# illini-robomaster/irmv_detection

Hardware: AMD Instinct MI355X
Metric: end-to-end FPS (preprocess→NMS→PnP) 640×640 YOLOv8n, 1/2/4/8 MI355X (higher is better)
Workload: dtype f16

## Files before the change

irmv_detection_amd/_build.py:

```python
from __future__ import annotations

import os
import shutil
import subprocess

_HERE = os.path.dirname(os.path.abspath(__file__))
CSRC = os.path.join(_HERE, "csrc")
LIB_DIR = os.path.join(_HERE, "lib")
LIB_PATH = os.path.join(LIB_DIR, "libirmv_hip.so")
INCLUDE = os.path.join(os.path.dirname(_HERE), "include")

SOURCES = [
    ("k_pre.hip", []),
    ("k_front.hip", []),
    ("k_c2f.hip", []),
    ("k_bneck.hip", []),
    ("k_kpt.hip", []),
    ("k_conv.hip", []),
    ("k_post.hip", ["-ffp-contract=off"]),
    ("k_light.hip", ["-ffp-contract=off"]),
    ("k_shuffle.hip", []),
    ("engine.cpp", ["-x", "hip"]),
]
COMMON = ["-O3", "-std=c++17", "-fPIC", "--offload-arch=gfx950", "-Wall", "-Wno-unused-function",
          "-mllvm", "-amdgpu-mfma-vgpr-form", "-I", INCLUDE]


def source_hash() -> str:
    import hashlib
    h = hashlib.sha256()
    names = sorted(set([s for s, _ in SOURCES] + ["irmv_common.hpp", "pnp_device.hpp", "numa.hpp"]))
    for n in names:
        pth = os.path.join(CSRC, n)
        if os.path.exists(pth):
            h.update(n.encode() + b"\0" + open(pth, "rb").read())
    h.update(open(os.path.join(INCLUDE, "irmv_hip.h"), "rb").read())
    h.update(" ".join(COMMON[:-2]).encode())
    for src, extra in SOURCES:
        h.update((src + " " + " ".join(extra)).encode())
    return h.hexdigest()


def hipcc() -> str:
    for cand in (shutil.which("hipcc"), "/opt/rocm/bin/hipcc"):
        if cand and os.path.exists(cand):
            return cand
    raise RuntimeError("hipcc not found: the HIP extension cannot be built")


def _stale(target: str, deps) -> bool:
    if not os.path.exists(target):
        return True
    t = os.path.getmtime(target)
    return any(os.path.getmtime(d) > t for d in deps)


COMM_PATH = os.path.join(LIB_DIR, "libirmv_comm.so")


def build_comm(force: bool = False, verbose: bool = False) -> str:
    os.makedirs(LIB_DIR, exist_ok=True)
    src = os.path.join(CSRC, "comm.cpp")
    deps = [src, os.path.join(INCLUDE, "irmv_comm.h"), os.path.join(INCLUDE, "irmv_hip.h"), __file__]
    if force or _stale(COMM_PATH, deps):
        rocm_lib = os.path.join(os.path.dirname(os.path.dirname(os.path.realpath(hipcc()))), "lib")
        cmd = [hipcc(), "-O2", "-std=c++17", "-fPIC", "-shared", "-Wall", "-I", INCLUDE, src, "-o", COMM_PATH,
               "-L", rocm_lib, "-lrccl", "-Wl,-rpath," + rocm_lib]
        if verbose:
            print(" ".join(cmd))
        subprocess.check_call(cmd)
    return COMM_PATH


def build(force: bool = False, verbose: bool = False) -> str:
    os.makedirs(LIB_DIR, exist_ok=True)
    headers = [os.path.join(CSRC, "irmv_common.hpp"), os.path.join(CSRC, "pnp_device.hpp"), os.path.join(CSRC, "numa.hpp"), os.path.join(INCLUDE, "irmv_hip.h"), __file__]
    objs = []
    cc = hipcc()
    for src, extra in SOURCES:
        sp = os.path.join(CSRC, src)
        obj = os.path.join(LIB_DIR, os.path.splitext(src)[0] + ".o")
        if force or _stale(obj, [sp] + headers):
            cmd = [cc] + COMMON + extra + os.environ.get("IRMV_EXTRA_HIPCC_FLAGS", "").split() + ["-c", sp, "-o", obj]
            if verbose:
                print(" ".join(cmd))
            subprocess.check_call(cmd)
        objs.append(obj)
    if force or _stale(LIB_PATH, objs):
        cmd = [cc, "-shared", "-fPIC", "--offload-arch=gfx950", "-o", LIB_PATH] + objs
        if verbose:
            print(" ".join(cmd))
        subprocess.check_call(cmd)
    return LIB_PATH


if __name__ == "__main__":
    print(build(force=False, verbose=True))
    print(build_comm(force=False, verbose=True))
# ... 1 lines not shown
```

irmv_detection_amd/csrc/engine.cpp:

```cpp
#include <hip/hip_runtime.h>

#include <algorithm>
#include <chrono>
#include <cmath>
#include <cstdio>
#include <cstring>
#include <fstream>
#include <map>
#include <mutex>
#include <set>
#include <memory>
#include <string>
#include <vector>

#include "../../include/irmv_hip.h"
#include "irmv_common.hpp"
#include "numa.hpp"

using namespace irmv;

constexpr int kLightPointsCap = 4096;

static thread_local std::string g_err;
static int fail(int code, const std::string &msg)
// ... 19 lines not shown
        snprintf(buf, sizeof buf, "irmv_hip 0.3 (gfx950; HIP runtime %d)", v);
    });
    return buf;
}
extern "C" int irmv_device_synchronize(int device)
{
    HIP_TRY(hipSetDevice(device));
    HIP_TRY(hipDeviceSynchronize());
    return IRMV_OK;
}
extern "C" int irmv_device_count(int *count)
{
    if (!count) return fail(IRMV_ERR_ARG, "count is null");
    HIP_TRY(hipGetDeviceCount(count));
    return IRMV_OK;
}

#pragma pack(push, 1)
struct BlobHeader { char magic[4]; uint32_t version, nc, nk, reg_max, n_layers, dtype, reserved; };
struct BlobLayer { char name[32]; uint32_t cin, cout, k, stride, act, pad; uint64_t w_off, b_off; };
#pragma pack(pop)

struct LayerW {
    std::string name;
    int cin, cout, k, stride, act;
    int groups;
    const uint16_t *w;
    const float *b;
};

static float half_bits_to_float(uint16_t h)
{
    const uint32_t sign = ((uint32_t)h & 0x8000u) << 16;
    uint32_t exp = (h >> 10) & 0x1fu, man = h & 0x3ffu, x;
    if (exp == 0) {
        if (man == 0) x = sign;
        else {
            int e = -1;
            do { e++; man <<= 1; } while (!(man & 0x400u));
            x = sign | ((uint32_t)(112 - e) << 23) | ((man & 0x3ffu) << 13);
        }
    } else if (exp == 31) x = sign | 0x7f800000u | (man << 13);
    else x = sign | ((exp + 112u) << 23) | (man << 13);
    float f;
    memcpy(&f, &x, 4);
    return f;
}

static uint16_t float_to_half_bits(float f)
{
    uint32_t x;
    memcpy(&x, &f, 4);
    const uint32_t sign = (x >> 16) & 0x8000u;
    x &= 0x7fffffffu;
    if (x >= 0x7f800000u) return (uint16_t)(sign | 0x7c00u | ((x > 0x7f800000u) ? 0x200u : 0u));
    if (x >= 0x477ff000u) return (uint16_t)(sign | 0x7c00u);
    if (x < 0x33000001u) return (uint16_t)sign;
    if (x < 0x38800000u) {
        const int shift = 126 - (int)(x >> 23);
        const uint32_t man = (x & 0x7fffffu) | 0x800000u;
        uint32_t h = man >> shift;
        const uint32_t rem = man & ((1u << shift) - 1u), half = 1u << (shift - 1);
        if (rem > half || (rem == half && (h & 1u))) h++;
        return (uint16_t)(sign | h);
    }
    uint32_t h = ((x >> 23) - 112u) << 10 | ((x >> 13) & 0x3ffu);
    const uint32_t rem = x & 0x1fffu;
    if (rem > 0x1000u || (rem == 0x1000u && (h & 1u))) h++;
    return (uint16_t)(sign | h);
}

struct Tensor {
    std::string name;
    void *base = nullptr;
    size_t slot_elems = 0;
    int H = 0, W = 0, C = 0;
    bool f32 = false;
    size_t esize() const { return f32 ? 4 : 2; }
    void *slot(int s) const { return static_cast<char *>(base) + (size_t)s * slot_elems * esize(); }
};

struct SegRef { int t = -1, coff = 0, C = 0, shift = 0; };

enum OpKind { OP_PRE, OP_CONV0, OP_CONV, OP_POOL, OP_NMS, OP_LIGHT, OP_FRONT, OP_C2F2, OP_C2F32, OP_DW, OP_SHUF, OP_SCAN, OP_BNECK, OP_KPT3 };

struct Op {
    OpKind kind;
    std::string layer;
    ConvCfg cfg{};
    ConvCfg cfg_one{};
    char kname_one[48] = {0};
    SegRef s0, s1;
    int Hin = 0, Win = 0, Hout = 0, Wout = 0, cin = 0, cout = 0, cout_pad = 0, ksteps = 0;
    int out_t = -1, out_coff = 0, res_t = -1, res_coff = 0;
    half_t *w_packed = nullptr;
    half_t *w_k16 = nullptr;
    half_t *w_lds[4] = {nullptr, nullptr, nullptr, nullptr};
    float *bias = nullptr;
    double flops = 0, bytes = 0;
    double w_bytes = 0;
    double out_bytes = 0;
    bool pair = false;
    int lane = 0;
    int level = -1;
    int signal = -1;
    char kname[48] = {0};
    int sub[4] = {-1, -1, -1, -1};
    int mode = 0;
    bool shortcut = false;
    int fuse_next = -1;
    bool fused_away = false;
    int group = -1;
    int bneck = -1;
    int kpt3 = -1;
};

struct GraphKey {
    int first, count;
    uint32_t flags;
    bool operator<(const GraphKey &o) const
    {
        return std::tie(first, count, flags) < std::tie(o.first, o.count, o.flags);
    }
};

struct SlotGroup {
    int first = 0, count = 0;
    hipEvent_t h2d = nullptr, out = nullptr;
    hipStream_t compute = nullptr;
    bool in_flight = false;
    bool async_up = false;
};

struct irmv_engine {
    irmv_engine_cfg cfg{};
    int nc = 0, nk = 0, A = 0, no = 0;
    int backbone = 0;
    int num_cus = 256;
    int numa_node = -1;
    bool numa_placed = false;
    struct HeadGroup { std::vector<int> members; int family = 0, nt = 1; ConvCfg cfg{}; char name[48] = {0}; };
    std::vector<HeadGroup> head_groups;
    bool post_keys_only = false;
    bool emit_scan = false;
    int emit_level_abase[3] = {0, 0, 0};
    bool split_scan = true;
    int *cand_counts = nullptr;
    int lvl_hw[3] = {0, 0, 0}, lvl_base[3] = {0, 0, 0};
    size_t frame_bytes = 0;
    hipStream_t stream = nullptr;
    hipStream_t extra_streams[7] = {nullptr, nullptr, nullptr, nullptr, nullptr, nullptr, nullptr};
    int num_streams = 1;
    hipStream_t h2d_stream = nullptr;
    std::map<std::pair<int, int>, SlotGroup> groups;
    std::vector<SlotGroup *> slot_owner;
    bool inline_copies = false;
    bool graph_upload = true;
    uint8_t *src_host = nullptr;
    int sync_launch = 0;
    hipStream_t enq_stream = nullptr;
    uint8_t *src_host_dev = nullptr;
    int upload_kernel_blocks = 256;
    uint8_t *src_dev = nullptr;
    uint8_t *rot_dev = nullptr;
    AxisTap *tap_x = nullptr, *tap_y = nullptr;
    std::vector<Tensor> tensors;
    std::map<std::string, int> tensor_idx;
    std::vector<Op> ops;
    std::vector<void *> dev_allocs;
    int head_t[3] = {-1, -1, -1};
    float *head_all = nullptr;
    PnpConst *pnp_dev = nullptr;
    long long *dbg_dev = nullptr;
    std::set<std::string> lazy_tensors;
    bool fused_front = false;
    int front_tiles_x = 0, front_tiles_y = 0, front_stage_bytes = 0, front_tile_y = kFrontTileY;
    int front_v[4] = {0, 0, 0, 0};
    int front_fastx = 0, front_fx_i0 = 0, front_fx_step = 2;
    bool classical = false;
    signed char *light_labels = nullptr;
    size_t light_pool = 0;
    short *light_points = nullptr, *light_hulls = nullptr;
    float *light_boxes = nullptr;
    DevDet *light_dets_dev = nullptr, *light_dets_host = nullptr;
    float *boxes = nullptr;
    unsigned long long *keys = nullptr;
    DevDet *dets_dev = nullptr, *dets_host = nullptr, *dets_host_dev = nullptr;
    DevFrameOut *fout_dev = nullptr, *fout_host = nullptr, *fout_host_dev = nullptr;
    bool zero_copy_results = false;
    half_t *conv0_w = nullptr;
    float *conv0_b = nullptr;
    PostArgs post{};
    std::map<GraphKey, hipGraphExec_t> graphs;
    double last_detect_ms = 0;
    std::vector<uint8_t> blob;
    std::vector<LayerW> layers;
    std::vector<std::vector<uint16_t>> dequant;
// ... 575 lines not shown
    TRY(new_tensor(e, "6", s16, s16, 128, false, &a6));
    TRY(new_tensor(e, "7", s32, s32, 256, false, &a7));
    TRY(new_tensor(e, "8", s32, s32, 256, false, &a8));
    TRY(new_tensor(e, "9.cat", s32, s32, 512, false, &s9));
    TRY(new_tensor(e, "9", s32, s32, 256, false, &a9));
    TRY(new_tensor(e, "12", s16, s16, 128, false, &a12));
    TRY(new_tensor(e, "15", s8, s8, 64, false, &a15));
    TRY(new_tensor(e, "16", s16, s16, 64, false, &a16));
    TRY(new_tensor(e, "18", s16, s16, 128, false, &a18));
    TRY(new_tensor(e, "19", s32, s32, 128, false, &a19));
    TRY(new_tensor(e, "21", s32, s32, 256, false, &a21));

    { Op op; op.kind = OP_PRE; op.layer = "preprocess"; snprintf(op.kname, sizeof op.kname, "preprocess");
      op.bytes = (double)e->frame_bytes + (double)net * net * 8; e->ops.push_back(op); }
    {
        const LayerW *l = find_layer(e, "model.0.conv");
        if (!l || l->cin != 3 || l->cout != 16 || l->k != 3 || l->stride != 2)
            return fail(IRMV_ERR_MODEL, "model.0.conv missing or not 3x3 s2 3->16");
        std::vector<uint16_t> w(2 * 64 * 8, 0);
        std::vector<float> b(16);
        for (int o = 0; o < 16; o++) b[o] = (float)((double)l->b[o] * (double)kActScale);
        for (int ks = 0; ks < 2; ks++)
            for (int lane = 0; lane < 64; lane++)
                for (int j = 0; j < 8; j++) {
                    const int g = lane >> 4, o = lane & 15;
                    const int kh = 2 * ks + (g >> 1), kw = 2 * (g & 1) + (j >> 2), ci = j & 3;
                    if (kh < 3 && kw < 3 && ci < 3) w[((size_t)ks * 64 + lane) * 8 + j] = l->w[(o * 9 + kh * 3 + kw) * 3 + ci];
                }
        TRY(dev_alloc(e, (void **)&e->conv0_w, w.size() * 2));
        TRY(dev_alloc(e, (void **)&e->conv0_b, b.size() * 4));
        HIP_TRY(hipMemcpy(e->conv0_w, w.data(), w.size() * 2, hipMemcpyHostToDevice));
        HIP_TRY(hipMemcpy(e->conv0_b, b.data(), b.size() * 4, hipMemcpyHostToDevice));
        Op op; op.kind = OP_CONV0; op.layer = "model.0.conv"; snprintf(op.kname, sizeof op.kname, "conv0_mfma");
        op.flops = 2.0 * s2 * s2 * 16 * 27;
        op.bytes = (double)net * net * 8 + (double)s2 * s2 * 32 + 27 * 16 * 2;
        e->ops.push_back(op);
    }
    TRY(add_conv(e, "model.1.conv", SegRef{a0, 0, 16, 0}, SegRef{}, s2, s2, a1, 0));
    {
        const Op &m1 = e->ops.back();
        if (!(m1.cfg.cin16 && m1.ksteps == 5 && m1.pair && m1.cout_pad == 32 && m1.out_coff == 0)) e->fused_front = false;
        if (e->fused_front) {
            Op op; op.kind = OP_FRONT; op.layer = "preprocess+model.0+model.1"; snprintf(op.kname, sizeof op.kname, "front_fused");
            op.flops = e->ops[1].flops + m1.flops;
            op.bytes = (double)e->frame_bytes + (double)s4 * s4 * 32 * 2;
            op.w_packed = m1.w_packed; op.bias = m1.bias; op.out_t = m1.out_t;
            for (Op &o : e->ops) o.fused_away = true;
            e->lazy_tensors.insert("input"); e->lazy_tensors.insert("0");
            e->ops.push_back(op);
        }
    }
    int p3 = a4, p4 = a6, p5 = a8;
    if (shuffle) {
        TRY(add_shuffle_down(e, "model.2", a1, 32, s4, s4, 64, a2));
        TRY(add_shuffle_unit(e, "model.3", a2, 64, s8, s8, a3));
        TRY(add_shuffle_down(e, "model.4", a3, 64, s8, s8, 128, a4));
        TRY(add_shuffle_unit(e, "model.5", a4, 128, s16, s16, a5));
        TRY(add_shuffle_unit(e, "model.6", a5, 128, s16, s16, a6));
        TRY(add_shuffle_down(e, "model.7", a6, 128, s16, s16, 256, a7));
        TRY(add_shuffle_unit(e, "model.8", a7, 256, s32, s32, a8));
        p3 = a3;
    } else {
    TRY(add_c2f(e, "model.2", SegRef{a1, 0, 32, 0}, SegRef{}, s4, s4, 32, 1, true, a2));
    {
        const int n = (int)e->ops.size();
        const Op &c1 = e->ops[n - 4], &m1 = e->ops[n - 3], &m2 = e->ops[n - 2], &c2 = e->ops[n - 1];
        bool ok = c1.cin == 32 && c1.cout == 32 && c1.cfg.ks == 1 && c1.pair && c1.ksteps == 1 &&
                  m1.cin == 16 && m1.cout == 16 && m1.cfg.cin16 && m1.ksteps == 5 && !m1.pair &&
                  m2.cin == 16 && m2.cout == 16 && m2.cfg.cin16 && m2.ksteps == 5 && !m2.pair && m2.res_t >= 0 &&
                  c2.cin == 48 && c2.cout == 32 && c2.cfg.ks == 1 && c2.pair && c2.ksteps == 2 &&
                  c1.cfg.act == 1 && m1.cfg.act == 1 && m2.cfg.act == 1 && c2.cfg.act == 1;
        if (const char *ff = getenv("IRMV_FUSED_C2F")) if (ff[0] == '0') ok = false;
        if (ok) {
            Op op; op.kind = OP_C2F2; op.layer = "model.2 (cv1+m.0+cv2)"; snprintf(op.kname, sizeof op.kname, "c2f2_fused");
            op.flops = c1.flops + m1.flops + m2.flops + c2.flops;
            op.bytes = 2.0 * (double)s4 * s4 * 32 * 2;
            for (int i = 0; i < 4; i++) { op.sub[i] = n - 4 + i; e->ops[n - 4 + i].fused_away = true; }
            op.s0 = c1.s0; op.out_t = c2.out_t;
            e->lazy_tensors.insert("model.2.cat"); e->lazy_tensors.insert("model.2.tmp");
            e->ops.push_back(op);
        }
    }
    TRY(add_conv(e, "model.3.conv", SegRef{a2, 0, 32, 0}, SegRef{}, s4, s4, a3, 0));
    TRY(add_c2f(e, "model.4", SegRef{a3, 0, 64, 0}, SegRef{}, s8, s8, 64, 2, true, a4));
    TRY(add_conv(e, "model.5.conv", SegRef{a4, 0, 64, 0}, SegRef{}, s8, s8, a5, 0));
    TRY(add_c2f(e, "model.6", SegRef{a5, 0, 128, 0}, SegRef{}, s16, s16, 128, 2, true, a6));
    TRY(add_conv(e, "model.7.conv", SegRef{a6, 0, 128, 0}, SegRef{}, s16, s16, a7, 0));
    TRY(add_c2f(e, "model.8", SegRef{a7, 0, 256, 0}, SegRef{}, s32, s32, 256, 1, true, a8));
    }
    TRY(add_conv(e, "model.9.cv1", SegRef{p5, 0, 256, 0}, SegRef{}, s32, s32, s9, 0));
    { Op op; op.kind = OP_POOL; op.layer = "model.9.m"; snprintf(op.kname, sizeof op.kname, "sppf_pool");
      op.bytes = (double)s32 * s32 * 128 * 2 * 4; e->ops.push_back(op); }
    TRY(add_conv(e, "model.9.cv2", SegRef{s9, 0, 512, 0}, SegRef{}, s32, s32, a9, 0));
    TRY(add_c2f(e, "model.12", SegRef{a9, 0, 256, 1}, SegRef{p4, 0, 128, 0}, s16, s16, 128, 1, false, a12));
    TRY(add_c2f(e, "model.15", SegRef{a12, 0, 128, 1}, SegRef{p3, 0, 64, 0}, s8, s8, 64, 1, false, a15));
    e->ops.back().signal = 0;
    TRY(add_conv(e, "model.16.conv", SegRef{a15, 0, 64, 0}, SegRef{}, s8, s8, a16, 0));
    TRY(add_c2f(e, "model.18", SegRef{a16, 0, 64, 0}, SegRef{a12, 0, 128, 0}, s16, s16, 128, 1, false, a18));
    e->ops.back().signal = 1;
    TRY(add_conv(e, "model.19.conv", SegRef{a18, 0, 128, 0}, SegRef{}, s16, s16, a19, 0));
    TRY(add_c2f(e, "model.21", SegRef{a19, 0, 128, 0}, SegRef{a9, 0, 256, 0}, s32, s32, 256, 1, false, a21));
    e->ops.back().signal = 2;

    const int P[3] = {a15, a18, a21}, PC[3] = {64, 128, 256}, PS[3] = {s8, s16, s32};
    int base = 0;
    for (int i = 0; i < 3; i++) {
        e->lvl_hw[i] = PS[i] * PS[i];
        e->lvl_base[i] = base;
        base += e->lvl_hw[i];
    }
    e->A = base;
    TRY(dev_alloc(e, (void **)&e->head_all, (size_t)S * e->A * kHeadRec * 4));
    HIP_TRY(hipMemset(e->head_all, 0, (size_t)S * e->A * kHeadRec * 4));
    for (int i = 0; i < 3; i++) {
        Tensor t;
        t.name = "head." + std::to_string(i);
        t.H = PS[i]; t.W = PS[i]; t.C = kHeadRec; t.f32 = true;
        t.slot_elems = (size_t)PS[i] * PS[i] * kHeadRec;
        t.base = e->head_all + (size_t)e->lvl_base[i] * S * kHeadRec;
        e->head_t[i] = (int)e->tensors.size();
        e->tensor_idx[t.name] = e->head_t[i];
        e->tensors.push_back(t);
    }
    const char *br[3] = {"cv2", "cv3", "cv4"};
    const int mid[3] = {64, 64, 16}, off[3] = {0, kClsOff, kKptOff};
    const int nbr = e->nk > 0 ? 3 : 2;
    {
        const char *mh = getenv("IRMV_MERGE_HEAD0");
        e->merge_head0 = stream_share(e, S) == 1 && !(mh && mh[0] == '0');
        if (mh && mh[0] == '1') e->merge_head0 = true;
        for (int i = 0; i < 3 && e->merge_head0; i++)
            for (int b = 0; b < nbr; b++) {
                const LayerW *l0 = find_layer(e, std::string("model.22.") + br[b] + "." + std::to_string(i) + ".0");
                if (!l0 || l0->k != 3 || l0->stride != 1 || l0->act != 1 || l0->cin != PC[i] || l0->cout != mid[b]) e->merge_head0 = false;
            }
    }
    const int coff0[3] = {0, 64, 128};
    int t_s0[3] = {-1, -1, -1};
    if (e->merge_head0) {
        const int cm = nbr == 3 ? 160 : 128;
        e->merged_w.reserve(3); e->merged_b.reserve(3);
        e->layers.reserve(e->layers.size() + 3);
        for (int i = 0; i < 3; i++) {
            const LayerW *src[3] = {nullptr, nullptr, nullptr};
            for (int b = 0; b < nbr; b++) src[b] = find_layer(e, std::string("model.22.") + br[b] + "." + std::to_string(i) + ".0");
            const size_t per_out = (size_t)9 * PC[i];
            e->merged_w.emplace_back((size_t)cm * per_out, (uint16_t)0);
            e->merged_b.emplace_back((size_t)cm, 0.f);
            for (int b = 0; b < nbr; b++) {
                memcpy(e->merged_w.back().data() + (size_t)coff0[b] * per_out, src[b]->w, (size_t)mid[b] * per_out * 2);
                memcpy(e->merged_b.back().data() + coff0[b], src[b]->b, (size_t)mid[b] * 4);
            }
            LayerW m;
            m.name = "model.22.s0." + std::to_string(i);
            m.cin = PC[i]; m.cout = cm; m.k = 3; m.stride = 1; m.act = 1;
            m.w = e->merged_w.back().data(); m.b = e->merged_b.back().data();
            e->layers.push_back(m);
            TRY(new_tensor(e, "22.s0." + std::to_string(i), PS[i], PS[i], cm, false, &t_s0[i]));
            TRY(add_conv(e, m.name, SegRef{P[i], 0, PC[i], 0}, SegRef{}, PS[i], PS[i], t_s0[i], 0));
            Op &mo = e->ops.back();
            const double real = nbr == 3 ? 144.0 : 128.0;
            mo.flops *= real / cm;
            mo.lane = 1; mo.level = i;
        }
    }
    for (int b = 0; b < nbr; b++)
// ... 760 lines not shown

static LightArgs light_args(const irmv_engine *e, int first)
{
    LightArgs a{};
    const irmv_engine_cfg &c = e->cfg;
    a.frames = e->src_dev + (size_t)first * e->frame_bytes;
    a.frame_bytes = e->frame_bytes;
    a.cols = c.src_width; a.rows = c.src_height; a.rotate180 = c.rotate180;
    a.dets = e->dets_dev + (size_t)first * c.max_det;
    a.max_det = c.max_det;
    a.num_dets = reinterpret_cast<const int *>(e->fout_dev + first);
    a.num_dets_stride = (int)(sizeof(DevFrameOut) / sizeof(int));
    a.n_boxes = 0;
    a.boxes = nullptr;
    a.labels = e->light_labels + (size_t)first * e->light_pool;
    a.label_pool = e->light_pool;
    a.points = e->light_points + (size_t)first * c.max_det * kLightPointsCap * 2;
    a.points_cap = kLightPointsCap;
    a.hulls = e->light_hulls + (size_t)first * c.max_det * kLightPointsCap * 4;
    a.binary_threshold = c.binary_threshold;
    a.light_min_ratio = c.light_min_ratio; a.light_max_ratio = c.light_max_ratio; a.light_max_angle = c.light_max_angle;
    a.min_small_cd = c.armor_min_small_center_distance; a.max_small_cd = c.armor_max_small_center_distance;
    a.min_large_cd = c.armor_min_large_center_distance; a.max_large_cd = c.armor_max_large_center_distance;
    a.pnp = e->pnp_dev;
    a.pnp_armor_size = c.armor_size;
    return a;
}

static PostArgs post_args(const irmv_engine *e, int first)
{
    PostArgs p = e->post;
    p.head_all = e->head_all;
    p.slots_total = e->cfg.num_slots;
    p.first = first;
    p.boxes = e->boxes + (size_t)first * e->A * 4;
    p.keys = e->keys + (size_t)first * e->A * e->nc;
    p.key_cap = e->A * e->nc;
    p.dets = (e->zero_copy_results ? e->dets_host_dev : e->dets_dev) + (size_t)first * e->cfg.max_det;
    p.fout = (e->zero_copy_results ? e->fout_host_dev : e->fout_dev) + first;
    if (p.dbg) p.dbg += (size_t)first * 16;
    p.counts = e->split_scan ? e->cand_counts + first : nullptr;
    return p;
}

static bool launch_c2f32_op(const irmv_engine *e, const Op &op, int first, int count, hipStream_t s)
{
    C2f32Args a{};
    const Tensor &ct = e->tensors[op.res_t];
    const Tensor &ot = e->tensors[op.out_t];
    if (op.sub[0] >= 0) {
        ConvArgs ca;
        fill_conv_args(e, e->ops[op.sub[0]], first, count, ca, false);
        a.s0 = ca.s0; a.s1 = ca.s1; a.cin1 = ca.Cin;
        a.w_cv1 = e->ops[op.sub[0]].w_packed; a.b_cv1 = e->ops[op.sub[0]].bias;
    } else {
        a.cin1 = 32;
    }
    a.cat = static_cast<half_t *>(ct.slot(first)); a.cat_ld = ct.C; a.prev_coff = 64;
    a.out = static_cast<half_t *>(ot.slot(first)); a.out_ld = ot.C;
    a.H = op.Hin; a.W = op.Win;
    a.tiles_x = (op.Win + kC2f32TileW - 1) / kC2f32TileW; a.tiles_y = (op.Hin + kC2f32TileH - 1) / kC2f32TileH;
    a.w_m1 = e->ops[op.sub[1]].w_packed; a.b_m1 = e->ops[op.sub[1]].bias;
    a.w_m2 = e->ops[op.sub[2]].w_packed; a.b_m2 = e->ops[op.sub[2]].bias;
    if (op.sub[3] >= 0) { a.w_cv2 = e->ops[op.sub[3]].w_packed; a.b_cv2 = e->ops[op.sub[3]].bias; }
    return launch_c2f32(op.mode, op.shortcut, a, count, s);
}

static int enqueue_step(irmv_engine *e, int first, int count, uint32_t flags, bool post_only, std::vector<EvRec> *ev)
{
    const int net = e->cfg.net_size;
    const bool capturing = (flags & 0x40000000u) != 0;
    const bool materialize = (flags & 0x20000000u) != 0;
    const PostArgs pa = post_args(e, first);
    (void)capturing;
    for (const Op &op : e->ops) {
        if (post_only && op.kind != OP_NMS && op.kind != OP_LIGHT && op.kind != OP_SCAN) continue;
        if (op.kind == OP_SCAN && e->emit_scan && !post_only) continue;
        const bool grouped = op.kind == OP_CONV && op.group >= 0 && count == 1 && !materialize && !post_only;
        if (grouped && e->head_groups[op.group].members[0] != (int)(&op - e->ops.data())) continue;
        const bool one_frame = count == 1 && !materialize && !post_only && e->bneck64;
        if (op.kind == OP_BNECK ? !one_frame : (op.bneck >= 0 && one_frame)) continue;
        const bool fused_kpt = !materialize && !post_only;
        if (op.kind == OP_KPT3 ? !fused_kpt : (op.kpt3 >= 0 && fused_kpt)) continue;
        if (materialize ? !(op.fused_away || op.fuse_next >= 0 || ((op.bneck >= 0 || op.kpt3 >= 0) && op.kind == OP_CONV)) : op.fused_away) continue;
        hipStream_t s = e->enq_stream ? e->enq_stream : e->stream;
        EvRec r{};
        r.op = (int)(&op - e->ops.data());
        if (ev) {
            HIP_TRY(hipEventCreate(&r.a));
            HIP_TRY(hipEventCreate(&r.b));
            HIP_TRY(hipEventRecord(r.a, s));
        }
        const bool once = op.kind == OP_LIGHT || (e->split_scan && (op.kind == OP_SCAN || op.kind == OP_NMS));
        const int reps = (ev && !once) ? (int)(flags & 0xffu) : 1;
        for (int rep = 0; rep < (reps > 0 ? reps : 1); rep++)
        switch (op.kind) {
        case OP_PRE: {
            PreArgs a;
            a.src = e->src_dev + (size_t)first * e->frame_bytes;
            a.dst = static_cast<half_t *>(e->tensors[e->tensor_idx.at("input")].slot(first));
            a.tx = e->tap_x; a.ty = e->tap_y;
            a.sw = e->cfg.src_width; a.sh = e->cfg.src_height; a.net = net; a.swap_rb = e->cfg.swap_rb;
            a.src_slot_bytes = e->frame_bytes;
            launch_preprocess(a, count, s);
            break;
        }
        case OP_FRONT: {
            FrontArgs a;
            a.src = e->src_dev + (size_t)first * e->frame_bytes;
            a.src_slot_bytes = e->frame_bytes;
            a.tx = e->tap_x; a.ty = e->tap_y;
            a.vx0 = e->front_v[0]; a.vx1 = e->front_v[1]; a.vy0 = e->front_v[2]; a.vy1 = e->front_v[3];
            a.sw = e->cfg.src_width; a.sh = e->cfg.src_height; a.net = net; a.swap_rb = e->cfg.swap_rb;
            a.fastx = e->front_fastx; a.fx_i0 = e->front_fx_i0; a.fx_step = e->front_fx_step;
            a.w0 = e->conv0_w; a.b0 = e->conv0_b;
            a.w1 = op.w_packed; a.b1 = op.bias;
            const Tensor &ot = e->tensors[op.out_t];
            a.out = static_cast<half_t *>(ot.slot(first));
            a.out_ld = ot.C;
            a.tiles_x = e->front_tiles_x; a.tiles_y = e->front_tiles_y; a.tile_y = e->front_tile_y;
            a.stage_bytes = e->front_stage_bytes;
            if (!launch_front(a, count, s)) return fail(IRMV_ERR_HIP, "fused front kernel: LDS request refused");
            break;
        }
        case OP_C2F2: {
            C2fArgs a;
            const Tensor &xt = e->tensors[op.s0.t], &ot = e->tensors[op.out_t];
            a.x = static_cast<const half_t *>(xt.slot(first)); a.x_ld = xt.C;
            a.out = static_cast<half_t *>(ot.slot(first)); a.out_ld = ot.C;
            a.S = xt.H; a.tiles = (xt.H + kC2fTile - 1) / kC2fTile;
            const Op &c1 = e->ops[op.sub[0]], &m1 = e->ops[op.sub[1]], &m2 = e->ops[op.sub[2]], &c2 = e->ops[op.sub[3]];
            a.w_cv1 = c1.w_packed; a.w_m1 = m1.w_packed; a.w_m2 = m2.w_packed; a.w_cv2 = c2.w_packed;
            a.b_cv1 = c1.bias; a.b_m1 = m1.bias; a.b_m2 = m2.bias; a.b_cv2 = c2.bias;
            launch_c2f2(a, count, s);
            break;
        }
        case OP_C2F32: {
            if (!launch_c2f32_op(e, op, first, count, s)) return fail(IRMV_ERR_ARG, "no fused C2f kernel for " + op.layer);
            break;
        }
        case OP_BNECK: {
            const Op &m1 = e->ops[op.sub[0]], &m2 = e->ops[op.sub[1]];
            const Tensor &ct = e->tensors[op.res_t];
            BneckArgs a{};
            a.yin = static_cast<const half_t *>(ct.slot(first)) + m1.s0.coff; a.yin_ld = ct.C;
            a.ynext = static_cast<half_t *>(ct.slot(first)) + m2.out_coff; a.ynext_ld = ct.C;
            a.cat = static_cast<const half_t *>(ct.slot(first)); a.cat_ld = ct.C;
            a.H = op.Hin; a.W = op.Win;
            a.tiles_x = (op.Win + kBneckTile - 1) / kBneckTile; a.tiles_y = (op.Hin + kBneckTile - 1) / kBneckTile;
            a.w_m1 = m1.w_lds[0]; a.b_m1 = m1.bias; a.w_m2 = m2.w_lds[0]; a.b_m2 = m2.bias;
            int ks2 = 6;
            if (op.sub[2] >= 0) {
                const Op &c2 = e->ops[op.sub[2]];
                const Tensor &ot = e->tensors[c2.out_t];
                a.out = static_cast<half_t *>(ot.slot(first)) + c2.out_coff; a.out_ld = ot.C;
                a.w_cv2 = c2.w_packed; a.b_cv2 = c2.bias;
                ks2 = c2.ksteps;
            }
            if (!launch_bneck64(op.mode, ks2, op.shortcut, a, count, s)) return fail(IRMV_ERR_ARG, "no fused bottleneck kernel for " + op.layer);
            break;
        }
        case OP_KPT3: {
            const Op &o0 = e->ops[op.sub[0]], &o1 = e->ops[op.sub[1]], &o2 = e->ops[op.sub[2]];
            const Tensor &xt = e->tensors[o0.s0.t], &ht = e->tensors[o2.out_t];
            Kpt3Args a{};
            a.x = static_cast<const half_t *>(xt.slot(first)) + o0.s0.coff; a.x_ld = xt.C;
            a.H = op.Hin; a.W = op.Win;
            a.tiles_x = (op.Win + kKpt3Tile - 1) / kKpt3Tile; a.tiles_y = (op.Hin + kKpt3Tile - 1) / kKpt3Tile;
            a.w1 = o0.w_lds[0]; a.b1 = o0.bias;
            a.w2 = o1.w_packed; a.b2 = o1.bias;
            a.w3 = o2.w_k16; a.b3 = o2.bias;
            a.out = static_cast<float *>(ht.slot(first)) + o2.out_coff; a.out_ld = ht.C;
            if (!launch_kpt3(a, op.cin, count, s)) return fail(IRMV_ERR_ARG, "no fused keypoint-branch kernel for " + op.layer);
            break;
        }
        case OP_DW: {
            DwArgs a;
            const Tensor &xt = e->tensors[op.s0.t], &ot = e->tensors[op.out_t];
            a.x = static_cast<const half_t *>(xt.slot(first)) + op.s0.coff; a.x_ld = xt.C;
            a.y = static_cast<half_t *>(ot.slot(first)) + op.out_coff; a.y_ld = ot.C;
            a.w = op.w_packed; a.b = op.bias;
            a.Hin = op.Hin; a.Win = op.Win; a.Hout = op.Hout; a.Wout = op.Wout; a.C = op.cout; a.stride = op.cfg.stride;
            launch_dwconv3x3(a, count, s);
            break;
        }
        case OP_SHUF: {
            ShufArgs a;
            const Tensor &at = e->tensors[op.s0.t], &bt = e->tensors[op.s1.t], &ot = e->tensors[op.out_t];
            a.a = static_cast<const half_t *>(at.slot(first)) + op.s0.coff; a.a_ld = at.C;
            a.b = static_cast<const half_t *>(bt.slot(first)) + op.s1.coff; a.b_ld = bt.C;
            a.out = static_cast<half_t *>(ot.slot(first)); a.out_ld = ot.C;
            a.bc = op.s0.C;
            a.pixels = (size_t)count * op.Hin * op.Win;
            launch_shuffle_cat(a, s);
            break;
        }
        case OP_CONV0: {
            Conv0Args a;
            a.x = static_cast<const half_t *>(e->tensors[e->tensor_idx.at("input")].slot(first));
            a.y = static_cast<half_t *>(e->tensors[e->tensor_idx.at("0")].slot(first));
            a.w = e->conv0_w; a.b = e->conv0_b; a.net = net; a.batch = count;
            launch_conv0(a, s);
            break;
        }
        case OP_CONV: {
            if (grouped) {
                if (!launch_head_group(e, e->head_groups[op.group], first, rep == (reps > 0 ? reps : 1) - 1 ? &pa : nullptr, s))
                    return fail(IRMV_ERR_ARG, std::string("grouped launch refused: ") + e->head_groups[op.group].name);
                break;
            }
            ConvArgs a;
            fill_conv_args(e, op, first, count, a, !materialize);
            if (e->emit_scan && !materialize && !post_only && is_cls_final_carrier(op) && rep == (reps > 0 ? reps : 1) - 1)
                scan_args_for(e, op, pa, a);
            const ConvCfg &cc = (count == 1 && stream_share(e, e->cfg.num_slots) > 1) ? op.cfg_one : op.cfg;
            if (!run_conv(op, cc, a, count, s)) return fail(IRMV_ERR_ARG, std::string("no conv kernel for ") + op.kname + " (" + op.layer + ")");
            break;
// ... 575 lines not shown
```

irmv_detection_amd/csrc/irmv_common.hpp:

```cpp
#pragma once

#include <hip/hip_runtime.h>

#include <cstdint>
#include <cstdlib>

namespace irmv {

typedef _Float16 half_t;
typedef _Float16 half8 __attribute__((ext_vector_type(8)));
typedef _Float16 half4 __attribute__((ext_vector_type(4)));
typedef float f32x4 __attribute__((ext_vector_type(4)));

constexpr float kActScale = 1.44269504088896341f;
constexpr float kActUnscale = 0.693147180559945309f;
typedef unsigned int u32x4_t __attribute__((ext_vector_type(4)));
__device__ __forceinline__ float silu_rcp(float y) { return __builtin_amdgcn_rcpf(1.0f + __builtin_amdgcn_exp2f(-y)); }
__device__ __forceinline__ unsigned int silu_pack2(float y0, float y1)
{
    const float r0 = silu_rcp(y0), r1 = silu_rcp(y1);
    unsigned int o;
    asm("v_fma_mixlo_f16 %0, %1, %2, 0" : "=v"(o) : "v"(y0), "v"(r0));
    asm("v_fma_mixhi_f16 %0, %1, %2, 0" : "+v"(o) : "v"(y1), "v"(r1));
    return o;
// ... 27 lines not shown
        tile = j % tiles;
    } else {
        const int r = id - full;
        image = (full / tiles) + r / tiles;
        tile = r % tiles;
    }
}

inline int xcd_image_order()
{
    const char *v = getenv("IRMV_XCD_IMAGES");
    return (v && v[0] == '0') ? 0 : 1;
}

inline int wres_stagger()
{
    const char *v = getenv("IRMV_WRES_STAGGER");
    return (v && v[0] == '0') ? 0 : 1;
}

constexpr int kHeadRec = 96;
constexpr int kClsOff = 64;
constexpr int kKptOff = 80;
constexpr int kCandCap = 8192;
constexpr int kMaxDetCap = 256;

struct AxisTap { int32_t i0, i1, w1, pad; };

struct PreArgs {
    const uint8_t *src;
    half_t *dst;
    const AxisTap *tx, *ty;
    int sw, sh, net, swap_rb;
    size_t src_slot_bytes;
};
void launch_preprocess(const PreArgs &a, int batch, hipStream_t s);
void launch_rotate180(const uint8_t *src, uint8_t *dst, int sw, int sh, hipStream_t s);
void launch_upload_frames(const uint8_t *src_host_mapped, uint8_t *dst, size_t bytes, int blocks, hipStream_t s);

struct Conv0Args {
    const half_t *x;
    half_t *y;
    const half_t *w;
    const float *b;
    int net, batch;
};
void launch_conv0(const Conv0Args &a, hipStream_t s);

constexpr int kFrontTileY = 4, kFrontTileX = 16;
constexpr int kFrontTileYDirect = 8;
constexpr int kFrontStageMax = 128 * 1024;
struct FrontArgs {
    const uint8_t *src;
    size_t src_slot_bytes;
    const AxisTap *tx, *ty;
    int vx0, vx1, vy0, vy1;
    int sw, sh, net, swap_rb;
    int fastx, fx_i0, fx_step;
    const half_t *w0;
    const float *b0;
    const half_t *w1;
    const float *b1;
    half_t *out;
    int out_ld;
    int tiles_x, tiles_y;
    int tile_y;
    int stage_bytes;
};
int front_min_stage_bytes(int tile_y = kFrontTileY);
bool front_prepare();
bool launch_front(const FrontArgs &a, int batch, hipStream_t s);

constexpr int kC2fTile = 16;
struct C2fArgs {
    const half_t *x;
    int x_ld;
    half_t *out;
    int out_ld;
    int S, tiles;
    const half_t *w_cv1, *w_m1, *w_m2, *w_cv2;
    const float *b_cv1, *b_m1, *b_m2, *b_cv2;
};
void launch_c2f2(const C2fArgs &a, int batch, hipStream_t s);

struct DwArgs {
    const half_t *x;
    int x_ld;
    half_t *y;
    int y_ld;
    const half_t *w;
    const float *b;
    int Hin, Win, Hout, Wout, C, stride;
};
void launch_dwconv3x3(const DwArgs &a, int batch, hipStream_t s);
struct ShufArgs {
    const half_t *a, *b;
    int a_ld, b_ld;
    half_t *out;
    int out_ld, bc;
    size_t pixels;
};
void launch_shuffle_cat(const ShufArgs &a, hipStream_t s);

struct ConvSeg {
    const half_t *p;
    int ld;
    int C;
    int shift;
};

constexpr int kC2f32TileH = 8, kC2f32TileW = 16;
struct C2f32Args {
    ConvSeg s0, s1;
    int cin1;
    half_t *cat;
    int cat_ld, prev_coff;
    half_t *out;
    int out_ld;
    int H, W, tiles_x, tiles_y;
    const half_t *w_cv1, *w_m1, *w_m2, *w_cv2;
    const float *b_cv1, *b_m1, *b_m2, *b_cv2;
};
size_t c2f32_lds_bytes(int mode);
bool launch_c2f32(int mode, bool shortcut, const C2f32Args &a, int batch, hipStream_t s);

constexpr int kBneckTile = 8;
struct BneckArgs {
    const half_t *yin;
    int yin_ld;
    half_t *ynext;
    int ynext_ld;
    const half_t *cat;
    int cat_ld;
    half_t *out;
    int out_ld;
    int H, W, tiles_x, tiles_y;
    const half_t *w_m1, *w_m2;
    const float *b_m1, *b_m2;
    const half_t *w_cv2;
    const float *b_cv2;
};
size_t bneck64_lds_bytes(int mode, int ks2);
bool launch_bneck64(int mode, int ks2, bool shortcut, const BneckArgs &a, int batch, hipStream_t s);

constexpr int kKpt3Tile = 10;
struct Kpt3Args {
    const half_t *x;
    int x_ld;
    int H, W, tiles_x, tiles_y;
    const half_t *w1;
    const float *b1;
    const half_t *w2;
    const float *b2;
    const half_t *w3;
    const float *b3;
    float *out;
    int out_ld;
};
bool kpt3_eligible(int cin);
bool launch_kpt3(const Kpt3Args &a, int cin, int batch, hipStream_t s);

struct ConvArgs {
    ConvSeg s0, s1;
    int Hin, Win;
    int Hout, Wout;
    int M;
// ... 140 lines not shown
```

Measured before the change: 62320.

## Fuse model.2 C2f block with stride-2 model.3 conv into one kernel

```diff
diff --git a/irmv_detection_amd/_build.py b/irmv_detection_amd/_build.py
--- a/irmv_detection_amd/_build.py
+++ b/irmv_detection_amd/_build.py
@@ -14,6 +14,7 @@
     ("k_pre.hip", []),
     ("k_front.hip", []),
     ("k_c2f.hip", []),
+    ("k_c2f2s2.hip", []),
     ("k_bneck.hip", []),
     ("k_kpt.hip", []),
     ("k_conv.hip", []),
diff --git a/irmv_detection_amd/csrc/engine.cpp b/irmv_detection_amd/csrc/engine.cpp
--- a/irmv_detection_amd/csrc/engine.cpp
+++ b/irmv_detection_amd/csrc/engine.cpp
@@ -125,7 +125,7 @@
 
 struct SegRef { int t = -1, coff = 0, C = 0, shift = 0; };
 
-enum OpKind { OP_PRE, OP_CONV0, OP_CONV, OP_POOL, OP_NMS, OP_LIGHT, OP_FRONT, OP_C2F2, OP_C2F32, OP_DW, OP_SHUF, OP_SCAN, OP_BNECK, OP_KPT3 };
+enum OpKind { OP_PRE, OP_CONV0, OP_CONV, OP_POOL, OP_NMS, OP_LIGHT, OP_FRONT, OP_C2F2, OP_C2F32, OP_DW, OP_SHUF, OP_SCAN, OP_BNECK, OP_KPT3, OP_C2F2S2 };
 
 struct Op {
     OpKind kind;
@@ -156,6 +156,7 @@
     int group = -1;
     int bneck = -1;
     int kpt3 = -1;
+    bool in_c2f2s2 = false;
 };
 
 struct GraphKey {
@@ -897,6 +898,27 @@
         }
     }
     TRY(add_conv(e, "model.3.conv", SegRef{a2, 0, 32, 0}, SegRef{}, s4, s4, a3, 0));
+    {
+        const int n = (int)e->ops.size();
+        const Op &c2 = e->ops[n - 2], &m3 = e->ops[n - 1];
+        bool ok = c2.kind == OP_C2F2 && m3.cin == 32 && m3.cout == 64 && m3.cout_pad == 64 && m3.cfg.ks == 3 && m3.cfg.stride == 2 &&
+                  m3.cfg.act == 1 && m3.pair && m3.w_lds[2] && m3.s1.C == 0 && m3.s0.t == c2.out_t && m3.s0.coff == 0 && m3.s0.shift == 0 &&
+                  m3.res_t < 0 && m3.out_coff == 0 && s4 % 2 == 0 && m3.Hout * 2 == s4 && m3.Wout * 2 == s4;
+        if (const char *ff = getenv("IRMV_FUSED_C2F2S2")) if (ff[0] == '0') ok = false;
+        if (getenv("IRMV_FORCE_W8")) ok = false;
+        if (ok) {
+            Op op; op.kind = OP_C2F2S2; op.layer = "model.2 (cv1+m.0+cv2) + model.3.conv"; snprintf(op.kname, sizeof op.kname, "c2f2s2_fused");
+            op.flops = c2.flops + m3.flops;
+            op.w_bytes = m3.w_bytes;
+            op.out_bytes = m3.out_bytes;
+            op.bytes = (double)s4 * s4 * 32 * 2 + m3.out_bytes + m3.w_bytes;
+            op.sub[0] = n - 2; op.sub[1] = n - 1;
+            op.s0 = c2.s0; op.out_t = m3.out_t;
+            e->ops[n - 2].in_c2f2s2 = true; e->ops[n - 1].in_c2f2s2 = true;
+            e->lazy_tensors.insert("2");
+            e->ops.push_back(op);
+        }
+    }
     TRY(add_c2f(e, "model.4", SegRef{a3, 0, 64, 0}, SegRef{}, s8, s8, 64, 2, true, a4));
     TRY(add_conv(e, "model.5.conv", SegRef{a4, 0, 64, 0}, SegRef{}, s8, s8, a5, 0));
     TRY(add_c2f(e, "model.6", SegRef{a5, 0, 128, 0}, SegRef{}, s16, s16, 128, 2, true, a6));
@@ -1823,6 +1845,8 @@
         if (op.kind == OP_BNECK ? !one_frame : (op.bneck >= 0 && one_frame)) continue;
         const bool fused_kpt = !materialize && !post_only;
         if (op.kind == OP_KPT3 ? !fused_kpt : (op.kpt3 >= 0 && fused_kpt)) continue;
+        const bool batched = count > 1 && !materialize && !post_only;
+        if (op.kind == OP_C2F2S2 ? !batched : (op.in_c2f2s2 && batched)) continue;
         if (materialize ? !(op.fused_away || op.fuse_next >= 0 || ((op.bneck >= 0 || op.kpt3 >= 0) && op.kind == OP_CONV)) : op.fused_away) continue;
         hipStream_t s = e->enq_stream ? e->enq_stream : e->stream;
         EvRec r{};
@@ -1874,6 +1898,21 @@
             a.w_cv1 = c1.w_packed; a.w_m1 = m1.w_packed; a.w_m2 = m2.w_packed; a.w_cv2 = c2.w_packed;
             a.b_cv1 = c1.bias; a.b_m1 = m1.bias; a.b_m2 = m2.bias; a.b_cv2 = c2.bias;
             launch_c2f2(a, count, s);
+            break;
+        }
+        case OP_C2F2S2: {
+            const Op &c2 = e->ops[op.sub[0]], &m3 = e->ops[op.sub[1]];
+            C2f2S2Args a;
+            const Tensor &xt = e->tensors[op.s0.t], &ot = e->tensors[op.out_t];
+            a.c.x = static_cast<const half_t *>(xt.slot(first)); a.c.x_ld = xt.C;
+            a.c.out = nullptr; a.c.out_ld = 0;
+            a.c.S = xt.H; a.c.tiles = (xt.H + kC2fTile - 1) / kC2fTile;
+            const Op &c1 = e->ops[c2.sub[0]], &m1 = e->ops[c2.sub[1]], &m2 = e->ops[c2.sub[2]], &cv2 = e->ops[c2.sub[3]];
+            a.c.w_cv1 = c1.w_packed; a.c.w_m1 = m1.w_packed; a.c.w_m2 = m2.w_packed; a.c.w_cv2 = cv2.w_packed;
+            a.c.b_cv1 = c1.bias; a.c.b_m1 = m1.bias; a.c.b_m2 = m2.bias; a.c.b_cv2 = cv2.bias;
+            a.out = static_cast<half_t *>(ot.slot(first)); a.out_ld = ot.C;
+            a.w3 = m3.w_lds[2]; a.b3 = m3.bias;
+            launch_c2f2s2(a, count, s);
             break;
         }
         case OP_C2F32: {
diff --git a/irmv_detection_amd/csrc/irmv_common.hpp b/irmv_detection_amd/csrc/irmv_common.hpp
--- a/irmv_detection_amd/csrc/irmv_common.hpp
+++ b/irmv_detection_amd/csrc/irmv_common.hpp
@@ -133,6 +133,14 @@
     const float *b_cv1, *b_m1, *b_m2, *b_cv2;
 };
 void launch_c2f2(const C2fArgs &a, int batch, hipStream_t s);
+struct C2f2S2Args {
+    C2fArgs c;
+    half_t *out;
+    int out_ld;
+    const half_t *w3;
+    const float *b3;
+};
+void launch_c2f2s2(const C2f2S2Args &a, int batch, hipStream_t s);
 
 struct DwArgs {
     const half_t *x;
diff --git a/irmv_detection_amd/csrc/k_c2f2s2.hip b/irmv_detection_amd/csrc/k_c2f2s2.hip
--- /dev/null
+++ b/irmv_detection_amd/csrc/k_c2f2s2.hip
@@ -0,0 +1,226 @@
+#include "irmv_common.hpp"
+
+namespace irmv {
+
+namespace {
+constexpr int T = kC2fTile;
+constexpr int T3 = T / 2;
+constexpr int OT = T + 1, ON = OT * OT;
+constexpr int XW = OT + 4;
+constexpr int TW = OT + 2;
+constexpr int HP = 32;
+constexpr int ZP = 80;
+
+__device__ __forceinline__ f32x4 bias4(const float *b) { return (f32x4){b[0], b[1], b[2], b[3]}; }
+typedef unsigned int u32x4 __attribute__((ext_vector_type(4)));
+__device__ __forceinline__ half8 as_h8(u32x4 v) { return __builtin_bit_cast(half8, v); }
+
+template <int RW>
+constexpr int region_tiles() { return RW + ((RW - 16) * RW + 15) / 16; }
+template <int RW>
+__device__ __forceinline__ bool region_px(int t, int r, int &ly, int &lx)
+{
+    constexpr int LC = RW - 16;
+    if (t < RW) { ly = t; lx = r; return true; }
+    const int q = (t - RW) * 16 + r;
+    const bool ok = q < LC * RW;
+    ly = ok ? q / LC : 0;
+    lx = ok ? 16 + q % LC : 0;
+    return ok;
+}
+}
+
+__global__ __launch_bounds__(256) void c2f2s2_kernel(C2f2S2Args a3, int batch, int xcd)
+{
+    const C2fArgs &a = a3.c;
+    __shared__ __attribute__((aligned(16))) uint8_t s_y1[XW * XW * HP];
+    __shared__ __attribute__((aligned(16))) uint8_t s_t[TW * TW * HP];
+    __shared__ __attribute__((aligned(16))) uint8_t s_z[ON * ZP];
+    __shared__ float s_bias[16 + 16 + 32];
+    const int tid = threadIdx.x, lane = tid & 63, wave = tid >> 6;
+    const int g = lane >> 4, r = lane & 15;
+    int tile_id, b;
+    tile_image(blockIdx.x, a.tiles * a.tiles, batch, xcd, tile_id, b);
+    const int tyi = tile_id / a.tiles, txi = tile_id - tyi * a.tiles;
+    const int py0 = tyi * T - 1, px0 = txi * T - 1;
+    const int S = a.S, S3 = S / 2;
+    const half8 zero8 = (half8){0, 0, 0, 0, 0, 0, 0, 0};
+
+    const half8 *w;
+    w = reinterpret_cast<const half8 *>(a.w_cv1) + lane;
+    const half8 Wc1[2] = {w[0], w[64]};
+    half8 Wm1[5], Wm2[5];
+    w = reinterpret_cast<const half8 *>(a.w_m1) + lane;
+#pragma unroll
+    for (int ks = 0; ks < 5; ks++) Wm1[ks] = w[ks * 64];
+    float bias_c1[8];
+#pragma unroll
+    for (int i = 0; i < 8; i++) bias_c1[i] = a.b_cv1[g * 8 + i];
+    if (tid < 16) { s_bias[tid] = a.b_m1[tid]; s_bias[16 + tid] = a.b_m2[tid]; }
+    else if (tid < 48) s_bias[16 + tid] = a.b_cv2[tid - 16];
+
+    {
+        constexpr int NTL = region_tiles<XW>(), PWV = NTL / 4;
+        static_assert(NTL % 4 == 0, "tiles split evenly over the waves");
+        const char *xbase = reinterpret_cast<const char *>(a.x);
+        const uint32_t img = (uint32_t)b * (uint32_t)(S * S);
+        u32x4 Bq[PWV];
+        int lyq[PWV], lxq[PWV];
+        bool okq[PWV];
+#pragma unroll
+        for (int i = 0; i < PWV; i++) {
+            okq[i] = region_px<XW>(wave + 4 * i, r, lyq[i], lxq[i]);
+            const int gy = py0 - 2 + lyq[i], gx = px0 - 2 + lxq[i];
+            const int gyc = gy < 0 ? 0 : (gy >= S ? S - 1 : gy), gxc = gx < 0 ? 0 : (gx >= S ? S - 1 : gx);
+            Bq[i] = *reinterpret_cast<const u32x4 *>(xbase + ((img + (uint32_t)(gyc * S + gxc)) * (uint32_t)a.x_ld + 8u * g) * 2u);
+        }
+#pragma unroll
+        for (int i = 0; i < PWV; i++) {
+            const int ly = lyq[i], lx = lxq[i];
+            const int gy = py0 - 2 + ly, gx = px0 - 2 + lx;
+            f32x4 acc0 = bias4(bias_c1), acc1 = bias4(bias_c1 + 4);
+            acc0 = __builtin_amdgcn_mfma_f32_16x16x32_f16(Wc1[0], as_h8(Bq[i]), acc0, 0, 0, 0);
+            acc1 = __builtin_amdgcn_mfma_f32_16x16x32_f16(Wc1[1], as_h8(Bq[i]), acc1, 0, 0, 0);
+            half8 o = zero8;
+            if ((unsigned)gy < (unsigned)S && (unsigned)gx < (unsigned)S)
+                o = silu_pack8(acc0[0], acc0[1], acc0[2], acc0[3], acc1[0], acc1[1], acc1[2], acc1[3]);
+            if (okq[i]) {
+                if (g >= 2) {
+                    *reinterpret_cast<half8 *>(s_y1 + (ly * XW + lx) * HP + (g - 2) * 16) = o;
+                } else if ((unsigned)(ly - 2) < (unsigned)OT && (unsigned)(lx - 2) < (unsigned)OT) {
+                    *reinterpret_cast<half8 *>(s_z + ((ly - 2) * OT + (lx - 2)) * ZP + g * 16) = o;
+                }
+            }
+        }
+    }
+    __syncthreads();
+
+    w = reinterpret_cast<const half8 *>(a.w_m2) + lane;
+#pragma unroll
+    for (int ks = 0; ks < 5; ks++) Wm2[ks] = w[ks * 64];
+
+    {
+        float bias[4];
+#pragma unroll
+        for (int i = 0; i < 4; i++) bias[i] = s_bias[g * 4 + i];
+        int toff[5];
+#pragma unroll
+        for (int ks = 0; ks < 5; ks++) {
+            const int tap = 2 * ks + (g >> 1), kh = tap / 3, kw = tap - kh * 3;
+            toff[ks] = tap < 9 ? (kh * XW + kw) * HP + 16 * (g & 1) : -1;
+        }
+        for (int t = wave; t < region_tiles<TW>(); t += 4) {
+            int ly, lx;
+            const bool mv = region_px<TW>(t, r, ly, lx);
+            const uint8_t *base = s_y1 + (ly * XW + lx) * HP;
+            f32x4 acc = bias4(bias);
+#pragma unroll
+            for (int ks = 0; ks < 5; ks++) {
+                half8 B = zero8;
+                if (toff[ks] >= 0) B = *reinterpret_cast<const half8 *>(base + toff[ks]);
+                acc = __builtin_amdgcn_mfma_f32_16x16x32_f16(Wm1[ks], B, acc, 0, 0, 0);
+            }
+            if (mv) {
+                const int gy = py0 - 1 + ly, gx = px0 - 1 + lx;
+                half4 o = (half4){0, 0, 0, 0};
+                if ((unsigned)gy < (unsigned)S && (unsigned)gx < (unsigned)S) o = silu_pack4(acc[0], acc[1], acc[2], acc[3]);
+                *reinterpret_cast<half4 *>(s_t + (ly * TW + lx) * HP + g * 8) = o;
+            }
+        }
+    }
+    __syncthreads();
+
+    w = reinterpret_cast<const half8 *>(a.w_cv2) + lane;
+    const half8 Wc2[2][2] = {{w[0], w[64]}, {w[128], w[192]}};
+
+    {
+        float bias[4];
+#pragma unroll
+        for (int i = 0; i < 4; i++) bias[i] = s_bias[16 + g * 4 + i];
+        int toff[5];
+#pragma unroll
+        for (int ks = 0; ks < 5; ks++) {
+            const int tap = 2 * ks + (g >> 1), kh = tap / 3, kw = tap - kh * 3;
+            toff[ks] = tap < 9 ? (kh * TW + kw) * HP + 16 * (g & 1) : -1;
+        }
+        for (int t = wave; t < region_tiles<OT>(); t += 4) {
+            int ly, lx;
+            const bool mv = region_px<OT>(t, r, ly, lx);
+            const uint8_t *base = s_t + (ly * TW + lx) * HP;
+            f32x4 acc = bias4(bias);
+#pragma unroll
+            for (int ks = 0; ks < 5; ks++) {
+                half8 B = zero8;
+                if (toff[ks] >= 0) B = *reinterpret_cast<const half8 *>(base + toff[ks]);
+                acc = __builtin_amdgcn_mfma_f32_16x16x32_f16(Wm2[ks], B, acc, 0, 0, 0);
+            }
+            const half4 rv = *reinterpret_cast<const half4 *>(s_y1 + ((ly + 2) * XW + lx + 2) * HP + g * 8);
+            half4 o;
+#pragma unroll
+            for (int i = 0; i < 4; i++) o[i] = silu_add_res(acc[i], (float)rv[i]);
+            if (mv) *reinterpret_cast<half4 *>(s_z + (ly * OT + lx) * ZP + 32 + g * 8) = o;
+        }
+    }
+    __syncthreads();
+
+    const int ch3 = (wave >> 1) * 32 + g * 8 + (wave & 1) * 4;
+    half8 W3[9];
+    w = reinterpret_cast<const half8 *>(a3.w3) + wave * 64 + lane;
+#pragma unroll
+    for (int tap = 0; tap < 9; tap++) W3[tap] = w[tap * 4 * 64];
+    const f32x4 b3 = *reinterpret_cast<const f32x4 *>(a3.b3 + ch3);
+
+    {
+        float bias[8];
+#pragma unroll
+        for (int i = 0; i < 8; i++) bias[i] = s_bias[32 + g * 8 + i];
+        for (int t = wave; t < region_tiles<OT>(); t += 4) {
+            int ly, lx;
+            const bool mv = region_px<OT>(t, r, ly, lx);
+            uint8_t *zp = s_z + (ly * OT + lx) * ZP;
+            const half8 B0 = g < 2 ? *reinterpret_cast<const half8 *>(zp + g * 16)
+                                   : *reinterpret_cast<const half8 *>(s_y1 + ((ly + 2) * XW + lx + 2) * HP + (g - 2) * 16);
+            half8 B1 = zero8;
+            if (g < 2) B1 = *reinterpret_cast<const half8 *>(zp + 32 + g * 16);
+            f32x4 acc0 = bias4(bias), acc1 = bias4(bias + 4);
+            acc0 = __builtin_amdgcn_mfma_f32_16x16x32_f16(Wc2[0][0], B0, acc0, 0, 0, 0);
+            acc1 = __builtin_amdgcn_mfma_f32_16x16x32_f16(Wc2[1][0], B0, acc1, 0, 0, 0);
+            acc0 = __builtin_amdgcn_mfma_f32_16x16x32_f16(Wc2[0][1], B1, acc0, 0, 0, 0);
+            acc1 = __builtin_amdgcn_mfma_f32_16x16x32_f16(Wc2[1][1], B1, acc1, 0, 0, 0);
+            const int gy = py0 + ly, gx = px0 + lx;
+            half8 o = zero8;
+            if ((unsigned)gy < (unsigned)S && (unsigned)gx < (unsigned)S)
+                o = silu_pack8(acc0[0], acc0[1], acc0[2], acc0[3], acc1[0], acc1[1], acc1[2], acc1[3]);
+            if (mv) *reinterpret_cast<half8 *>(zp + g * 16) = o;
+        }
+    }
+    __syncthreads();
+
+    {
+        f32x4 acc[4] = {b3, b3, b3, b3};
+#pragma unroll
+        for (int tap = 0; tap < 9; tap++) {
+            const int kh = tap / 3, kw = tap - kh * 3;
+            half8 B[4];
+#pragma unroll
+            for (int mt = 0; mt < 4; mt++)
+                B[mt] = *reinterpret_cast<const half8 *>(s_z + ((2 * (2 * mt + (r >> 3)) + kh) * OT + 2 * (r & 7) + kw) * ZP + g * 16);
+#pragma unroll
+            for (int mt = 0; mt < 4; mt++) acc[mt] = __builtin_amdgcn_mfma_f32_16x16x32_f16(W3[tap], B[mt], acc[mt], 0, 0, 0);
+        }
+        half_t *out = a3.out + (size_t)b * S3 * S3 * a3.out_ld + ch3;
+#pragma unroll
+        for (int mt = 0; mt < 4; mt++) {
+            const int oy = tyi * T3 + 2 * mt + (r >> 3), ox = txi * T3 + (r & 7);
+            if (oy < S3 && ox < S3)
+                *reinterpret_cast<half4 *>(out + ((size_t)oy * S3 + ox) * a3.out_ld) = silu_pack4(acc[mt][0], acc[mt][1], acc[mt][2], acc[mt][3]);
+        }
+    }
+}
+
+void launch_c2f2s2(const C2f2S2Args &a, int batch, hipStream_t s)
+{
+    hipLaunchKernelGGL(c2f2s2_kernel, dim3(a.c.tiles * a.c.tiles * batch), dim3(256), 0, s, a, batch, xcd_image_order());
+}
+
+}
```

Result: no change. 62690 (median of 6 runs) (+0.6%).
